# mmp/pbrt-v4

Hardware: AMD Instinct MI355X
Metric: Msamples/sec (whole node), 1920x1080 at fixed spp (higher is better)
Workload: dtype f32; 1 GPU; San Miguel 1080p 256spp (BASELINE.json configs[2]) on the sanmiguel-like stand-in at the SURVEY 8(d) spec: 10001008 unique triangles in 2000 meshes, 60 % of them in 200 object-instance definitions (two-level BVH), 10 % alpha-cut, 1k^2 image textures, diffuse / coated diffuse / dielectric / conductor, sun + 2k^2 image sky + 500 emitters, maxdepth 5, zsobol; step = 1 sample index x 1920x1080; spp=321, samples_per_pass=64, partition=single GPU

## Files before the change

### pbrt-v4_amd/csrc/hip/wf_backend.hip

```cpp
#include <hip/hip_runtime.h>
#include <array>

#include <climits>
#include <cstdarg>
#include <cstdio>
#include <cstring>
#include <algorithm>
#include <atomic>
#include <map>
#include <string>
#include <thread>
#include <type_traits>
#include <utility>
#include <vector>

#pragma clang attribute push(__attribute__((uninitialized)), apply_to = variable(is_local))
#include "../common/wf_kernels.h"
#include "../common/wf_kat.h"
#pragma clang attribute pop
#include "wf_traverse.h"

using namespace wf;

static thread_local char g_err[512] = "";
// ... 20 lines not shown
using ClosestWalkFn = void (*)(const SceneView, WorkState, FastBVH, int, SpillArea, int *, int, const int *);
using ShadowWalkFn = void (*)(const SceneView, WorkState, FastBVH, SpillArea, int *, int, const int *);
using TrTraceFn = void (*)(const SceneView, WorkState, FastBVH, int, SpillArea);
using TraceClosestFn = void (*)(const SceneView, FastBVH, int, const float *, wf_hit_record *, SpillArea);
using TraceAnyFn = void (*)(const SceneView, FastBVH, int, const float *, int32_t *, SpillArea);
struct WalkKernels {
    ClosestWalkFn closest = nullptr;
    ShadowWalkFn shadow = nullptr;
    ClosestWalkFn closestGen = nullptr;
    ShadowWalkFn shadowGen = nullptr;
    int grid = 1024, gridShadow = 1024, gridGen = 1024, gridShadowGen = 1024;
    TrTraceFn trTrace = nullptr;
    TraceClosestFn traceClosest = nullptr;
    TraceAnyFn traceAny = nullptr;
};

struct wf_ctx {
    int device = 0;
    hipStream_t stream = nullptr;
    std::vector<void *> allocs;
    SceneView svHost{};
    const SceneView *svDev = nullptr;
    WorkState ws{};
    int maxQueueSize = 0;
    int *stackSpill = nullptr;
    int spillRows = 0;
    int *dbgWords = nullptr;
    SpillArea spillArea() const { return SpillArea{stackSpill, spillRows, dbgWords}; }
    FastBVH fast{};
    bool fastOk = false;
    hipStream_t stream2 = nullptr;
    hipEvent_t evFork = nullptr, evJoin = nullptr;
    bool retracePending = false, deferJoin = false;
    int trWavefront = -1;
    bool cursorDirty[2] = {false, false};
    bool mediumLean = false;
    bool portalLights = false;
    bool leanShade = false;
    bool leanType[WF_MAT_NTYPES] = {};
    bool rareLights = false;
    int genMode = 0;
    bool deferGeneral = false;
    int genTri = 0;
    int nestedAnimated = 0;
    bool animFast = false;
    WalkKernels walk;
    int cursorChunk = 2;
    int cursorChunkShadow = 2;
    int32_t *probeCursor = nullptr;
    bool matPresent[WF_MAT_NTYPES] = {};
    int W = 0, H = 0;
    int maxDepth = 5;
    float sceneBounds[6] = {};
    bool sceneLoaded = false, queuesAllocated = false;
    int profile = 0;
    struct Ev { std::string name; hipEvent_t a, b; };
    std::vector<Ev> events;
    std::vector<hipEvent_t> eventPool;
    int passY0 = INT_MIN;
    int passStep = 1, passSamples = 1;
    bool pixelMajor = true;
    bool countTraversal = false;
    bool traceLaunch = false;
};

template <typename T>
static int devAlloc(wf_ctx *c, T **p, size_t n) {
    void *d = nullptr;
    size_t bytes = std::max<size_t>(n, 1) * sizeof(T);
    HIPCHK(hipMalloc(&d, bytes));
    HIPCHK(hipMemsetAsync(d, 0, bytes, c->stream));
    c->allocs.push_back(d);
    *p = (T *)d;
    return 0;
}
template <typename T>
static int devUpload(wf_ctx *c, const T **p, const T *src, size_t n) {
    T *d = nullptr;
    if (int e = devAlloc(c, &d, n)) return e;
    if (n && src) HIPCHK(hipMemcpyAsync(d, src, n * sizeof(T), hipMemcpyHostToDevice, c->stream));
    *p = d;
    return 0;
}

template <typename T>
static int devUpload(wf_ctx *c, wf::GPtr<const T> *p, const T *src, size_t n) {
    const T *d = nullptr;
    if (int e = devUpload(c, &d, src, n)) return e;
    *p = d;
    return 0;
}

template <bool VIA_SELF>
__device__ inline const SceneView &SvOf(const SceneView &a) { return VIA_SELF ? *a.self : a; }
__global__ void __launch_bounds__(BLOCK) k_reset(WorkState ws, unsigned mask, int statSlot, int statCounter) {
    if (threadIdx.x == 0 && blockIdx.x == 0) {
        if (statSlot >= 0) ws.stats[statSlot] += (unsigned long long)ws.counters[(statCounter) * CNT_STRIDE];
// ... 1082 lines not shown
}

struct Prof {
    wf_ctx *c;
    hipEvent_t a = nullptr, b = nullptr;
    const char *name;
    bool on;
    hipStream_t s;
    Prof(wf_ctx *c, const char *name, hipStream_t onStream = nullptr) : c(c), name(name), s(onStream ? onStream : c->stream) {
        if (c->traceLaunch) { fprintf(stderr, "[wf] launch %s\n", name); fflush(stderr); }
        on = c->profile == 1 || (c->profile == 2 && (strncmp(name, "Intersect", 9) == 0 || strcmp(name, "Route hits") == 0 || strstr(name, "Material") != nullptr ||
                                                      strncmp(name, "Sample medium", 13) == 0));
        if (!on) return;
        auto get = [&]() {
            hipEvent_t e;
            if (!c->eventPool.empty()) { e = c->eventPool.back(); c->eventPool.pop_back(); }
            else (void)hipEventCreate(&e);
            return e;
        };
        a = get(); b = get();
        (void)hipEventRecord(a, s);
    }
    ~Prof() {
        if (c->traceLaunch) {
            hipError_t e = hipStreamSynchronize(s);
            if (e != hipSuccess) { fprintf(stderr, "[wf] %s: %s\n", name, hipGetErrorString(e)); fflush(stderr); }
        }
        if (!on) return;
        (void)hipEventRecord(b, s);
        c->events.push_back({name, a, b});
    }
};

#define LAUNCH(name, kernel, grid, ...)                                                    \
    do {                                                                                   \
        Prof prof_(ctx, name);                                                             \
        hipLaunchKernelGGL(kernel, dim3(grid), dim3(BLOCK), 0, ctx->stream, __VA_ARGS__);  \
    } while (0)

#define LAUNCHT(name, kernel, grid, ...)                                                   \
    do {                                                                                   \
        Prof prof_(ctx, name);                                                             \
        hipLaunchKernelGGL(kernel, dim3(grid), dim3(TBLOCK), 0, ctx->stream, __VA_ARGS__); \
    } while (0)

static int statDepth(int depth) { return depth < 63 ? depth : 63; }

__global__ void k_pack_grid_corners(const float *v, int nx, int ny, int nz, float *out) {
    const size_t cells = (size_t)(nx + 1) * (ny + 1) * (nz + 1);
    for (size_t c = (size_t)blockIdx.x * blockDim.x + threadIdx.x; c < cells; c += (size_t)gridDim.x * blockDim.x) {
        const int cx = (int)(c % (size_t)(nx + 1)), cy = (int)((c / (size_t)(nx + 1)) % (size_t)(ny + 1)), cz = (int)(c / ((size_t)(nx + 1) * (ny + 1)));
        const int ix = cx - 1, iy = cy - 1, iz = cz - 1;
        float *o = out + 8 * wf::GridCornerIndex(nx, ny, cx, cy, cz);
        o[0] = wf::GridLookupI(v, nx, ny, nz, ix, iy, iz);         o[1] = wf::GridLookupI(v, nx, ny, nz, ix + 1, iy, iz);
        o[2] = wf::GridLookupI(v, nx, ny, nz, ix, iy + 1, iz);     o[3] = wf::GridLookupI(v, nx, ny, nz, ix + 1, iy + 1, iz);
        o[4] = wf::GridLookupI(v, nx, ny, nz, ix, iy, iz + 1);     o[5] = wf::GridLookupI(v, nx, ny, nz, ix + 1, iy, iz + 1);
        o[6] = wf::GridLookupI(v, nx, ny, nz, ix, iy + 1, iz + 1); o[7] = wf::GridLookupI(v, nx, ny, nz, ix + 1, iy + 1, iz + 1);
    }
}
static void useDevice(const wf_ctx *ctx) { (void)hipSetDevice(ctx->device); }
static int checkReady(wf_ctx *ctx) {
    if (!ctx) return fail(-1, "null context");
    if (!ctx->sceneLoaded) return fail(-1, "no scene uploaded");
    if (!ctx->queuesAllocated) return fail(-1, "queues not allocated (wf_queues_alloc)");
    useDevice(ctx);
    return 0;
}

struct FastDepths { int top = 0, def = 0, maxLeafInstances = 0; };
struct TopPrim {
    float b[6];
    int kind;
    int idx;
};
struct TopTreeBuilder {
    std::vector<TopPrim> &P;
    std::vector<wf_bvh_node> &out;
// ... 762 lines not shown
            const float(*mi)[4] = in.render_from_instance.mInv;
            double oI[3], dI[3];
            for (int a = 0; a < 3; ++a) {
                oI[a] = (double)mi[a][0] * o[0] + (double)mi[a][1] * o[1] + (double)mi[a][2] * o[2] + (double)mi[a][3];
                dI[a] = (double)mi[a][0] * dir[0] + (double)mi[a][1] * dir[1] + (double)mi[a][2] * dir[2];
            }
            const wf_instance_def &def = d->instance_defs[in.def];
            for (int k = def.first_prim; k < def.first_prim + def.n_prims; ++k)
                if (d->bvh_prims[k] < d->n_triangles) check(d->bvh_prims[k], ii, oI, dI);
        }
    }
    out[7] = cw.entries;
    out[3] = cw.nodesVisited;
    return 0;
}

constexpr int SCRATCH_PRIME_WORDS = 896;
__global__ void k_scratch_prime(int *out, int n) {
    volatile int buf[SCRATCH_PRIME_WORDS];
    for (int i = 0; i < n; ++i) buf[(i * 131) % SCRATCH_PRIME_WORDS] = i;
    out[threadIdx.x] = buf[(n * 7) % SCRATCH_PRIME_WORDS];
}
int wf_ctx_create(int device, wf_ctx **out) {
    if (!out) return fail(-1, "null out");
    int ndev = 0;
    HIPCHK(hipGetDeviceCount(&ndev));
    if (ndev <= 0) return fail(-1, "no HIP device visible: libwfhip has no CPU fallback");
    if (device < 0 || device >= ndev) return fail(-1, "device %d out of range (0..%d)", device, ndev - 1);
    HIPCHK(hipSetDevice(device));
    wf_ctx *c = new wf_ctx();
    c->device = device;
    HIPCHK(hipStreamCreateWithFlags(&c->stream, hipStreamNonBlocking));
    HIPCHK(hipStreamCreateWithFlags(&c->stream2, hipStreamNonBlocking));
    HIPCHK(hipEventCreateWithFlags(&c->evFork, hipEventDisableTiming));
    HIPCHK(hipEventCreateWithFlags(&c->evJoin, hipEventDisableTiming));
    c->traceLaunch = getenv("WF_TRACE_LAUNCH") != nullptr;
    if (const char *e = getenv("WF_SCRATCH_PRIME"); !e || atoi(e) != 0) {
        int *tmp = nullptr;
        HIPCHK(hipMalloc(&tmp, 64 * sizeof(int)));
        hipLaunchKernelGGL(k_scratch_prime, dim3(1), dim3(64), 0, c->stream, tmp, 8);
        hipLaunchKernelGGL(k_scratch_prime, dim3(1), dim3(64), 0, c->stream2, tmp, 8);
        HIPCHK(hipStreamSynchronize(c->stream));
        HIPCHK(hipStreamSynchronize(c->stream2));
        HIPCHK(hipFree(tmp));
    }
    *out = c;
    return 0;
}

int wf_ctx_destroy(wf_ctx *ctx) {
    if (!ctx) return 0;
    (void)hipSetDevice(ctx->device);
    (void)hipStreamSynchronize(ctx->stream);
    for (void *p : ctx->allocs) (void)hipFree(p);
    for (auto &e : ctx->events) { (void)hipEventDestroy(e.a); (void)hipEventDestroy(e.b); }
    for (auto e : ctx->eventPool) (void)hipEventDestroy(e);
    (void)hipStreamDestroy(ctx->stream);
    if (ctx->stream2) (void)hipStreamDestroy(ctx->stream2);
    if (ctx->evFork) (void)hipEventDestroy(ctx->evFork);
    if (ctx->evJoin) (void)hipEventDestroy(ctx->evJoin);
    delete ctx;
    return 0;
}

int wf_sync(wf_ctx *ctx) {
    if (!ctx) return fail(-1, "null context");
    useDevice(ctx);
    HIPCHK(hipStreamSynchronize(ctx->stream));
    HIPCHK(hipGetLastError());
    if (ctx->dbgWords) {
        int overflow = 0;
        HIPCHK(hipMemcpy(&overflow, ctx->dbgWords + 1, sizeof(int), hipMemcpyDeviceToHost));
        if (overflow) return fail(-1, "traversal stack overflow: a walk needed more than %d + %d node-stack entries (results are incomplete)", TSTACK, ctx->spillRows);
        int unresolved = 0;
        HIPCHK(hipMemcpy(&unresolved, ctx->dbgWords + 6, sizeof(int), hipMemcpyDeviceToHost));
        if (unresolved & 1) return fail(-1, "a near-tie re-walk found no hit where the production walk had one (results are incomplete)");
        if (unresolved & 2) return fail(-1, "a near-tie queue entry failed its validation (ray index, bound or launch tag): results are incomplete");
        int fatal = 0;
        HIPCHK(hipMemcpy(&fatal, ctx->dbgWords + 7, sizeof(int), hipMemcpyDeviceToHost));
        if (fatal) return fail(-1, "%s", FatalMessage(fatal));
        if (getenv("WF_DEBUG_DRAIN")) {
            int h[8];
            HIPCHK(hipMemcpy(h, ctx->dbgWords, sizeof(h), hipMemcpyDeviceToHost));
            fprintf(stderr, "[drain] spilled %d, re-walks %d, pushes %d, repeated re-walks %d, unresolved %d\n", h[0], h[2], h[4], h[5], h[6]);
#if WF_WALK_STATS
            unsigned long long c[16];
            HIPCHK(hipMemcpy(c, ctx->dbgWords + 8, sizeof(c), hipMemcpyDeviceToHost));
            const char *ph[4] = {"interior", "leaf", "transition", "refill"};
            for (int k = 0; k < 2; ++k)
                for (int q = 0; q < 4; ++q)
                    fprintf(stderr, "[walk stats] %s %-26s wave iterations %llu, lanes %llu (%.1f per iteration)\n", k ? "any-hit" : "closest", ph[q], c[k * 8 + 2 * q], c[k * 8 + 2 * q + 1],
// ... 275 lines not shown
                    st.pop_back();
                    best = std::max(best, dep);
                    if (d->bvh_nodes[i].nprims == 0) { st.push_back({i + 1, dep + 1}); st.push_back({d->bvh_nodes[i].offset, dep + 1}); }
                }
                return best;
            };
            int depthTop = d->n_bvh_nodes > 0 ? treeDepth(0) : 0, depthDef = 0;
            for (int k = 0; k < d->n_instance_defs; ++k) depthDef = std::max(depthDef, treeDepth(d->instance_defs[k].bvh_root));
            const int needRef = depthTop + (ctx->nestedAnimated > 0 ? 2 : 1) * depthDef + 4;
            const int needFast = 3 * fdep.top + fdep.maxLeafInstances + 3 * fdep.def + 6;
            const int rows = std::max(std::max(needRef - std::min(STACK_LDS, TSTACK), needFast - TSTACK), STACK_MAX - std::min(STACK_LDS, TSTACK));
            if (rows > 2048) return fail(-1, "BVH too deep for the traversal stacks (depth %d + %d)", depthTop, depthDef);
            if ((e = devAlloc(ctx, &ctx->stackSpill, (size_t)rows * MAX_GRID * BLOCK))) return e;
            ctx->spillRows = rows;
            if ((e = devAlloc(ctx, &ctx->dbgWords, (size_t)8 + 32))) return e;
            HIPCHK(hipMemset(ctx->dbgWords, 0, (8 + 32) * sizeof(int)));
        }
        if (ctx->fastOk) {
            if ((e = devUpload(ctx, &ctx->fast.nodes, qn.data(), qn.size()))) return e;
            if ((e = devUpload(ctx, &ctx->fast.tris, lt.data(), lt.size()))) return e;
            if ((e = devUpload(ctx, &ctx->fast.defs, fdefs.data(), fdefs.size()))) return e;
            if ((e = devUpload(ctx, &ctx->fast.subs, fsubs.data(), fsubs.size()))) return e;
            const bool big = qn.size() * sizeof(QNode) + lt.size() * sizeof(LeafTri) > ((size_t)256 << 20);
            ctx->cursorChunk = big ? 3 : 2;
            ctx->cursorChunkShadow = big ? 1 : 2;
            ctx->fast.instances = ctx->svHost.instances;
            HIPCHK(hipStreamSynchronize(ctx->stream));
        }
        if (getenv("WF_NO_FAST")) ctx->fastOk = false;
        ctx->animFast = d->n_animated > 0 && ctx->fastOk && ctx->genMode <= 1 && ctx->svHost.nInstances > 0 && !(getenv("WF_ANIM_FAST") && atoi(getenv("WF_ANIM_FAST")) == 0);
        if (d->n_animated > 0 && !ctx->animFast) ctx->fastOk = false;
        if ((e = PickWalkKernels(ctx))) return e;
        if ((e = devAlloc(ctx, &ctx->probeCursor, (size_t)1))) return e;
    }
    if ((e = devAlloc(ctx, &ctx->ws.film, (size_t)ctx->W * ctx->H * 4))) return e;
    ctx->ws.filmSpectral = nullptr;
    ctx->ws.filmGBuffer = nullptr;
    if (d->film.type == WF_FILM_GBUFFER && (e = devAlloc(ctx, &ctx->ws.filmGBuffer, (size_t)ctx->W * ctx->H))) return e;
    if (d->film.type == WF_FILM_SPECTRAL) {
        if (d->film.n_buckets < 1 || d->film.n_buckets > 4096 || !(d->film.lambda_max > d->film.lambda_min)) return fail(-1, "spectral film: bad bucket count / wavelength range");
        if ((e = devAlloc(ctx, &ctx->ws.filmSpectral, (size_t)ctx->W * ctx->H * 2 * d->film.n_buckets))) return e;
    }
    if ((e = devAlloc(ctx, &ctx->ws.stats, (size_t)(129 + 16)))) return e;
    if ((e = devAlloc(ctx, &ctx->ws.trav, (size_t)8))) return e;
    if ((e = devAlloc(ctx, &ctx->ws.counters, (size_t)CNT_COUNT * CNT_STRIDE))) return e;
    {
        SceneView *dev = nullptr;
        if ((e = devAlloc(ctx, &dev, (size_t)1))) return e;
        ctx->svHost.self = dev;
        ctx->svHost.fatal = ctx->dbgWords ? ctx->dbgWords + 7 : nullptr;
        HIPCHK(hipMemcpyAsync(dev, &ctx->svHost, sizeof(SceneView), hipMemcpyHostToDevice, ctx->stream));
        ctx->svDev = dev;
    }
    ctx->fast.sv = ctx->svDev;
    HIPCHK(hipStreamSynchronize(ctx->stream));
    ctx->sceneLoaded = true;
    return 0;
}

int wf_ctx_query(wf_ctx *ctx, const char *key, int64_t *value) {
    if (!ctx || !key || !value) return fail(-1, "wf_ctx_query: null argument");
    if (!ctx->sceneLoaded) return fail(-1, "no scene uploaded");
    const std::string k = key;
    if (k == "fast_ok") *value = ctx->fastOk;
    else if (k == "gen_mode") *value = ctx->genMode;
    else if (k == "gen_tri") *value = ctx->genTri;
    else if (k == "defer_general") *value = ctx->deferGeneral;
    else if (k == "anim_fast") *value = ctx->animFast;
    else if (k == "lean_shade") *value = ctx->leanShade;
    else if (k == "rare_lights") *value = ctx->rareLights;
    else if (k == "medium_lean") *value = ctx->mediumLean;
    else if (k.rfind("lean_type_", 0) == 0 && atoi(key + 10) >= 0 && atoi(key + 10) < WF_MAT_NTYPES) *value = ctx->leanType[atoi(key + 10)];
    else if (k == "instances") *value = ctx->svHost.nInstances;
    else if (k == "nested_animated") *value = ctx->nestedAnimated;
    else return fail(-1, "wf_ctx_query: unknown key '%s'", key);
    return 0;
}

int wf_aggregate_bounds(wf_ctx *ctx, float out_bounds[6]) {
    if (!ctx || !ctx->sceneLoaded) return fail(-1, "no scene uploaded");
    useDevice(ctx);
    for (int i = 0; i < 6; ++i) out_bounds[i] = ctx->sceneBounds[i];
    return 0;
}

static int allocRayQueue(wf_ctx *c, RayQueueV *q, size_t n) {
    int e;
    if ((e = devAlloc(c, &q->o, n)) || (e = devAlloc(c, &q->d, n)) || (e = devAlloc(c, &q->beta, n)) || (e = devAlloc(c, &q->r_u, n)) ||
        (e = devAlloc(c, &q->r_l, n)) || (e = devAlloc(c, &q->ctx0, n)) || (e = devAlloc(c, &q->ctx1, n)) || (e = devAlloc(c, &q->ctx2, n)) ||
        (e = devAlloc(c, &q->meta, n)))
        return e;
    return 0;
}

int wf_queues_alloc(wf_ctx *ctx, int pixels_per_pass, int samples_per_pass) {
    if (!ctx || !ctx->sceneLoaded) return fail(-1, "no scene uploaded");
    useDevice(ctx);
    if (ctx->queuesAllocated) return fail(-1, "queues already allocated");
    if (pixels_per_pass <= 0 || samples_per_pass <= 0) return fail(-1, "pixels_per_pass and samples_per_pass must be positive");
    if ((long long)pixels_per_pass * samples_per_pass > (1ll << 30)) return fail(-1, "queue capacity %lld too large", (long long)pixels_per_pass * samples_per_pass);
    if (pixels_per_pass % ctx->W != 0) return fail(-1, "pixels_per_pass must be a whole number of scanlines (width %d)", ctx->W);
    HIPCHK(hipSetDevice(ctx->device));
    const int max_queue_size = pixels_per_pass * samples_per_pass;
    const size_t n = (size_t)max_queue_size;
    WorkState &ws = ctx->ws;
    ws.maxQueueSize = max_queue_size;
    ws.pixelsPerPass = pixels_per_pass;
    ws.samplesPerPass = samples_per_pass;
    if (ws.stripCount < 1) { ws.stripRank = 0; ws.stripCount = 1; ws.stripHeight = 1; ws.localRows = ctx->H; }
    ctx->passSamples = 1;
    if (const char *e = getenv("WF_PIXEL_MAJOR")) ctx->pixelMajor = atoi(e) != 0;
    ctx->ws.slotStride = ctx->pixelMajor ? 1 : 0;
    ctx->passStep = 1;
    int e;
    if ((e = devAlloc(ctx, &ws.filterWeight, n)) || (e = devAlloc(ctx, &ws.pPixel, n)) || (e = devAlloc(ctx, &ws.lambda, n)) ||
        (e = devAlloc(ctx, &ws.lambdaPdf, n)) || (e = devAlloc(ctx, &ws.L, n)) || (e = devAlloc(ctx, &ws.cameraRayWeight, n)) ||
        (e = devAlloc(ctx, &ws.samples0, n)) || (e = devAlloc(ctx, &ws.samples1, n)))
        return e;
    if (ctx->svHost.film.type == WF_FILM_GBUFFER &&
        ((e = devAlloc(ctx, &ws.vsP, n)) || (e = devAlloc(ctx, &ws.vsN, n)) || (e = devAlloc(ctx, &ws.vsNs, n)) || (e = devAlloc(ctx, &ws.vsDpdx, n)) ||
         (e = devAlloc(ctx, &ws.vsDpdy, n)) || (e = devAlloc(ctx, &ws.vsAlbedo, n))))
        return e;
    ws.sampleTops = nullptr;
    if (ctx->svHost.sampler.type == WF_SAMPLER_ZSOBOL && 2 * ctx->svHost.sampler.nBase4Digits <= 32 && !getenv("WF_NO_SAMPLE_TOPS") &&
        !ctx->svHost.haveSubsurface)
        if ((e = devAlloc(ctx, &ws.sampleTops, (size_t)5 * pixels_per_pass))) return e;
    if ((e = allocRayQueue(ctx, &ws.rq[0], n)) || (e = allocRayQueue(ctx, &ws.rq[1], n))) return e;
    if (ctx->svHost.haveMedia) {
        if (getenv("WF_TR_WAVEFRONT")) ctx->trWavefront = atoi(getenv("WF_TR_WAVEFRONT"));
        if ((e = devAlloc(ctx, &ws.trO, n)) || (e = devAlloc(ctx, &ws.trD, n)) || (e = devAlloc(ctx, &ws.trT, n)) || (e = devAlloc(ctx, &ws.trRu, n)) ||
            (e = devAlloc(ctx, &ws.trRl, n)) || (e = devAlloc(ctx, &ws.trRng, n)) || (e = devAlloc(ctx, &ws.trQ[0], n)) || (e = devAlloc(ctx, &ws.trQ[1], n)))
            return e;
        if ((e = devAlloc(ctx, &ws.hitT, n)) || (e = devAlloc(ctx, &ws.mediumSampleQ, n)) || (e = devAlloc(ctx, &ws.mediumScatterQ, n)) || (e = devAlloc(ctx, &ws.mediumRouteQ, n)) ||
            (e = devAlloc(ctx, &ws.scatterP, n)) || (e = devAlloc(ctx, &ws.sq.medium, n)))
            return e;
    }
    if (ctx->svHost.haveMix && ((e = devAlloc(ctx, &ws.mixMat, n)) || (e = devAlloc(ctx, &ws.mixQ, n)))) return e;
    if (ctx->svHost.haveSubsurface && ((e = devAlloc(ctx, &ws.samples2, n)) || (e = devAlloc(ctx, &ws.bssrdfQ, n)) || (e = devAlloc(ctx, &ws.sssQ, n)))) return e;
    if ((e = devAlloc(ctx, &ws.hit, n)) || (e = devAlloc(ctx, &ws.escapedQ, n)) || (e = devAlloc(ctx, &ws.hitLightQ, n)) || (e = devAlloc(ctx, &ws.retraceQ, n)) || (e = devAlloc(ctx, &ws.retraceQ64, n))) return e;
    if ((e = devAlloc(ctx, &ws.deferQ, n))) return e;
    HIPCHK(hipMemset(ws.retraceQ64, 0xff, (size_t)n * sizeof(unsigned long long)));
    if (ctx->svHost.nInstances > 0 && (e = devAlloc(ctx, &ws.hitInst, n))) return e;
    for (int m = 0; m < WF_MAT_NTYPES; ++m)
        if ((e = devAlloc(ctx, &ws.matQ[m], ctx->matPresent[m] ? n : (size_t)1))) return e;
    if ((e = devAlloc(ctx, &ws.sq.o, n)) || (e = devAlloc(ctx, &ws.sq.d, n)) || (e = devAlloc(ctx, &ws.sq.Ld, n)) ||
        (e = devAlloc(ctx, &ws.sq.r_u, n)) || (e = devAlloc(ctx, &ws.sq.r_l, n)))
        return e;
    if (ctx->svHost.haveAnimated && (e = devAlloc(ctx, &ws.pathTime, n))) return e;
    {
        int planes = 0;
        for (int m = 1; m < WF_MAT_NTYPES; ++m) if (ctx->matPresent[m]) planes = std::max(planes, NeePlanes(m));
        if (planes > 0 && (e = devAlloc(ctx, &ws.neeRec, n * (size_t)planes))) return e;
    }
    if ((e = devAlloc(ctx, &ws.routeCode, n))) return e;
    ctx->maxQueueSize = max_queue_size;
    ctx->queuesAllocated = true;
    return 0;
}

int wf_set_pass_samples(wf_ctx *ctx, int sample_step, int n_samples) {
    if (int e = checkReady(ctx)) return e;
    if (n_samples < 1 || n_samples > ctx->ws.samplesPerPass) return fail(-1, "n_samples %d outside 1..%d", n_samples, ctx->ws.samplesPerPass);
    if (sample_step < 1) return fail(-1, "sample_step must be >= 1");
    ctx->passStep = sample_step;
    ctx->passSamples = n_samples;
    ctx->ws.slotStride = ctx->pixelMajor ? n_samples : 0;
    return 0;
}

int wf_set_strips(wf_ctx *ctx, int rank, int count, int height, int *local_rows) {
    if (!ctx || !ctx->sceneLoaded) return fail(-1, "no scene uploaded");
    useDevice(ctx);
    if (count < 1 || rank < 0 || rank >= count || height < 1) return fail(-1, "wf_set_strips: rank %d of %d, height %d", rank, count, height);
    int rows = 0;
    for (int y = 0; y < ctx->H; ++y) rows += (y / height) % count == rank;
    ctx->ws.stripRank = rank; ctx->ws.stripCount = count; ctx->ws.stripHeight = height; ctx->ws.localRows = count > 1 ? rows : ctx->H;
    if (local_rows) *local_rows = ctx->ws.localRows;
    return 0;
}

int wf_film_clear(wf_ctx *ctx) {
    if (!ctx || !ctx->sceneLoaded) return fail(-1, "no scene uploaded");
    useDevice(ctx);
    HIPCHK(hipMemsetAsync(ctx->ws.film, 0, (size_t)ctx->W * ctx->H * 4 * sizeof(double), ctx->stream));
    if (ctx->ws.filmGBuffer) HIPCHK(hipMemsetAsync(ctx->ws.filmGBuffer, 0, (size_t)ctx->W * ctx->H * sizeof(wf_gbuffer_pixel), ctx->stream));
    if (ctx->ws.filmSpectral) HIPCHK(hipMemsetAsync(ctx->ws.filmSpectral, 0, (size_t)ctx->W * ctx->H * 2 * ctx->svHost.film.n_buckets * sizeof(double), ctx->stream));
    HIPCHK(hipMemsetAsync(ctx->ws.stats, 0, (129 + 16) * sizeof(unsigned long long), ctx->stream));
    HIPCHK(hipMemsetAsync(ctx->ws.trav, 0, 8 * sizeof(unsigned long long), ctx->stream));
    return 0;
}

int wf_reset_ray_queue(wf_ctx *ctx, int which) {
    if (int e = checkReady(ctx)) return e;
    LAUNCH("Reset ray queue", k_reset, 1, ctx->ws, 1u << (CNT_RAY0 + (which & 1)), -1, 0);
    return 0;
}
int wf_reset_stage_queues(wf_ctx *ctx, int depth) {
    if (int e = checkReady(ctx)) return e;
    const int cur = depth & 1;
    unsigned mask = (1u << (CNT_RAY0 + (cur ^ 1))) | (1u << CNT_ESCAPED) | (1u << CNT_HITLIGHT);
    for (int m = 0; m < WF_MAT_NTYPES; ++m) mask |= 1u << (CNT_MAT0 + m);
    mask |= (1u << CNT_MEDIUM_SAMPLE) | (1u << CNT_MEDIUM_SCATTER) | (1u << CNT_MIX) | (1u << CNT_RETRACE) | (1u << CNT_BSSRDF) | (1u << CNT_SSS);
    mask |= (1u << CNT_RETRACE_HEAD) | (1u << CNT_WAVES_DONE) | (1u << CNT_CURSOR) | (1u << CNT_MEDIUM_ROUTE) | (1u << CNT_DEFER) | (1u << CNT_CURSOR_MEDIUM);
    LAUNCH("Reset queues before tracing rays", k_reset, 1, ctx->ws, mask, 1 + statDepth(depth), CNT_RAY0 + cur);
    ctx->cursorDirty[0] = false;
    return 0;
}
int wf_gen_camera_rays(wf_ctx *ctx, int y0, int sample_index) {
    if (int e = checkReady(ctx)) return e;
    ctx->passY0 = y0;
    if (ctx->ws.sampleTops) LAUNCH("Sampler index prefixes", k_sample_tops, gridFor(5 * ctx->ws.pixelsPerPass), ctx->svHost, ctx->ws, y0, 0);
    if (ctx->svHost.camera.type == WF_CAMERA_REALISTIC)
        LAUNCH("Reset ray queue", k_reset, 1, ctx->ws, 1u << CNT_RAY0, -1, 0);
    LAUNCH("Generate camera rays", (ctx->svHost.camera.anim.actually_animated ? k_gen_camera_rays<true> : k_gen_camera_rays<false>), gridFor(ctx->maxQueueSize), ctx->svHost, ctx->ws, y0, sample_index,
           ctx->passStep, ctx->passSamples);
    LAUNCH("Update camera ray stats", k_reset, 1, ctx->ws, 0u, 0, CNT_RAY0);
    return 0;
}
int wf_gen_ray_samples(wf_ctx *ctx, int depth, int sample_index) {
    if (int e = checkReady(ctx)) return e;
    const bool tops = ctx->ws.sampleTops != nullptr && ctx->passY0 != INT_MIN;
    if (tops) LAUNCH("Sampler index prefixes", k_sample_tops, gridFor(5 * ctx->ws.pixelsPerPass), ctx->svHost, ctx->ws, ctx->passY0, 6 + 7 * depth);
    LAUNCH("Generate ray samples - ZSobolSampler", k_gen_ray_samples, gridFor(ctx->maxQueueSize), ctx->svHost, ctx->ws, depth & 1, sample_index, ctx->passStep,
           tops ? depth : -1);
    return 0;
}
static int JoinRetrace(wf_ctx *ctx) {
    if (!ctx->retracePending) return 0;
    HIPCHK(hipStreamWaitEvent(ctx->stream, ctx->evJoin, 0));
    ctx->retracePending = false;
    return 0;
}
int wf_intersect_closest(wf_ctx *ctx, int depth) {
    if (int e = checkReady(ctx)) return e;
    const bool anim = ctx->svHost.haveAnimated;
    if (ctx->countTraversal)
// ... 86 lines not shown
                                               "DiffuseTransmissionMaterial + BxDF eval (Basic tex)", "CoatedDiffuseMaterial + BxDF eval (Basic tex)",
                                               "CoatedConductorMaterial + BxDF eval (Basic tex)", "SubsurfaceMaterial + BxDF eval (Basic tex)", "HairMaterial + BxDF eval (Basic tex)",
                                               "MeasuredMaterial + BxDF eval (Basic tex)"};
    if (material_type == WF_MAT_INTERFACE) return 0;
    if (material_type < 0 || material_type >= WF_MAT_NTYPES) return fail(-1, "material type %d has no HIP kernel", material_type);
    const bool tex = ctx->svHost.texNeedsFootprint != 0;
    const bool vs = ctx->svHost.film.type == WF_FILM_GBUFFER || ctx->svHost.camera.anim.actually_animated || ctx->svHost.haveAnimated ||
                    (ctx->svHost.haveCurves && ctx->svHost.haveQuadricAlpha);
    {
        Prof prof_(ctx, names[material_type]);
        const int v = vs ? 3 : (!ctx->leanType[material_type] ? 2 : (tex ? 1 : 0));
        kMatShade[material_type][v](ctx->stream, g, &ctx->svHost, &ctx->ws, cur);
    }
    {
        static const char *neeNames[WF_MAT_NTYPES] = {"", "DiffuseMaterial: next-event estimation", "ConductorMaterial: next-event estimation", "DielectricMaterial: next-event estimation",
                                                      "ThinDielectricMaterial: next-event estimation", "DiffuseTransmissionMaterial: next-event estimation",
                                                      "CoatedDiffuseMaterial: next-event estimation", "CoatedConductorMaterial: next-event estimation",
                                                      "SubsurfaceMaterial: next-event estimation", "HairMaterial: next-event estimation", "MeasuredMaterial: next-event estimation"};
        Prof prof_(ctx, neeNames[material_type]);
        kMatNee[material_type][ctx->rareLights ? 1 : 0](ctx->stream, g, &ctx->svHost, &ctx->ws);
    }
    return 0;
}
int wf_eval_material(wf_ctx *ctx, int material_type, int depth) {
    if (int e = checkReady(ctx)) return e;
    return EvalMaterial(ctx, material_type, depth);
}
static int EvalMaterials(wf_ctx *ctx, int depth) {
    for (int m = 1; m < WF_MAT_NTYPES; ++m)
        if (ctx->matPresent[m])
            if (int e = EvalMaterial(ctx, m, depth)) return e;
    return 0;
}
int wf_intersect_shadow(wf_ctx *ctx, int depth) {
    if (int e = checkReady(ctx)) return e;
    const bool anim = ctx->svHost.haveAnimated;
    if (ctx->countTraversal)
        LAUNCH("Intersect shadow", (anim ? k_intersect_shadow<true, true> : k_intersect_shadow<true, false>), gridFor(ctx->maxQueueSize), ctx->svHost, ctx->ws, ctx->stackSpill);
    else if (ctx->fastOk) {
        const WalkKernels &k = ctx->walk;
        int *cursor = ctx->ws.counters + CNT_CURSOR_SHADOW * CNT_STRIDE;
        if (ctx->cursorDirty[1]) HIPCHK(hipMemsetAsync(cursor, 0, sizeof(int), ctx->stream));
        ctx->cursorDirty[1] = true;
        LAUNCHT("Intersect shadow", k.shadow, k.gridShadow, ctx->svHost, ctx->ws, ctx->fast, ctx->spillArea(), cursor, ctx->cursorChunkShadow, (const int *)nullptr);
        if (k.shadowGen)
            LAUNCHT("Intersect shadow: rays that met a general primitive", k.shadowGen, k.gridShadowGen, ctx->svHost, ctx->ws, ctx->fast, ctx->spillArea(), (int *)nullptr, ctx->cursorChunkShadow, (const int *)ctx->ws.deferQ);
    } else
        LAUNCH("Intersect shadow", (anim ? k_intersect_shadow<false, true> : k_intersect_shadow<false, false>), gridFor(ctx->maxQueueSize), ctx->svHost, ctx->ws, ctx->stackSpill);
    LAUNCH("Reset shadowRayQueue", k_reset, 1, ctx->ws, (1u << CNT_SHADOW) | (1u << CNT_CURSOR_SHADOW) | (1u << CNT_DEFER_SHADOW), 65 + statDepth(depth), CNT_SHADOW);
    ctx->cursorDirty[1] = false;
    return 0;
}
int wf_subsurface_probe(wf_ctx *ctx, int depth) {
    if (int e = checkReady(ctx)) return e;
    if (!ctx->svHost.haveSubsurface) return 0;
    (void)depth;
    LAUNCH("Get BSSRDF and enqueue probe ray", k_subsurface_probe, gridFor(ctx->maxQueueSize), ctx->svHost, ctx->ws);
    return 0;
}
int wf_intersect_one_random(wf_ctx *ctx) {
    if (int e = checkReady(ctx)) return e;
    if (!ctx->svHost.haveSubsurface) return 0;
    LAUNCH("Intersect one random (subsurface probe)", (ctx->svHost.haveAnimated ? k_intersect_one_random<true> : k_intersect_one_random<false>), gridFor(ctx->maxQueueSize), ctx->svHost, ctx->ws, ctx->stackSpill);
    return 0;
}
int wf_subsurface_scatter(wf_ctx *ctx, int depth) {
    if (int e = checkReady(ctx)) return e;
    if (!ctx->svHost.haveSubsurface) return 0;
    LAUNCH("Handle out-scattering after SSS", k_subsurface_scatter, gridFor(ctx->maxQueueSize), ctx->svHost, ctx->ws, depth & 1);
    return 0;
}
int wf_update_film(wf_ctx *ctx) {
    if (int e = checkReady(ctx)) return e;
    if (ctx->ws.slotStride > 0 && ctx->ws.slotStride == ctx->passSamples && ctx->passSamples <= FILM_MAX_SLOTS && ctx->svHost.film.type == WF_FILM_RGB)
        LAUNCH("Update film", k_update_film_pm, std::min(4096, (ctx->ws.pixelsPerPass + FILM_PIX - 1) / FILM_PIX), ctx->svHost, ctx->ws, ctx->passSamples);
    else
        LAUNCH("Update film", k_update_film, gridFor(ctx->ws.pixelsPerPass), ctx->svHost, ctx->ws, ctx->passSamples);
    return 0;
}

int wf_render_pass(wf_ctx *ctx, int y0, int sample_index) {
    if (int e = checkReady(ctx)) return e;
    int e;
    if ((e = wf_reset_ray_queue(ctx, 0))) return e;
    if ((e = wf_gen_camera_rays(ctx, y0, sample_index))) return e;
    for (int depth = 0; true; ++depth) {
        if ((e = wf_reset_stage_queues(ctx, depth))) return e;
        ctx->deferJoin = ctx->fastOk && !ctx->countTraversal && !ctx->svHost.haveMix;
        if ((e = wf_intersect_closest(ctx, depth))) { ctx->deferJoin = false; return e; }
        ctx->deferJoin = false;
        if ((e = wf_gen_ray_samples(ctx, depth, sample_index))) return e;
        if ((e = JoinRetrace(ctx))) return e;
        if ((e = wf_medium_sample(ctx, depth))) return e;
        if ((e = wf_handle_escaped(ctx, depth))) return e;
        if ((e = wf_handle_emissive(ctx, depth))) return e;
        if (depth == ctx->maxDepth) break;
        if ((e = EvalMaterials(ctx, depth))) return e;
        if ((e = ctx->svHost.haveMedia ? wf_intersect_shadow_tr(ctx, depth) : wf_intersect_shadow(ctx, depth))) return e;
        if (ctx->svHost.haveSubsurface) {
            if ((e = wf_subsurface_probe(ctx, depth)) || (e = wf_intersect_one_random(ctx)) || (e = wf_subsurface_scatter(ctx, depth))) return e;
            if ((e = ctx->svHost.haveMedia ? wf_intersect_shadow_tr(ctx, depth) : wf_intersect_shadow(ctx, depth))) return e;
        }
    }
    return wf_update_film(ctx);
}

int wf_film_download(wf_ctx *ctx, double *dst) {
    if (!ctx || !ctx->sceneLoaded) return fail(-1, "no scene uploaded");
    useDevice(ctx);
    HIPCHK(hipMemcpyAsync(dst, ctx->ws.film, (size_t)ctx->W * ctx->H * 4 * sizeof(double), hipMemcpyDeviceToHost, ctx->stream));
    HIPCHK(hipStreamSynchronize(ctx->stream));
    return 0;
}
int wf_film_spectral_download(wf_ctx *ctx, double *dst) {
    if (!ctx || !ctx->sceneLoaded) return fail(-1, "no scene uploaded");
    useDevice(ctx);
    if (!ctx->ws.filmSpectral) return fail(-1, "wf_film_spectral_download: the scene's film is not a spectral film");
    HIPCHK(hipMemcpyAsync(dst, ctx->ws.filmSpectral, (size_t)ctx->W * ctx->H * 2 * ctx->svHost.film.n_buckets * sizeof(double), hipMemcpyDeviceToHost, ctx->stream));
    HIPCHK(hipStreamSynchronize(ctx->stream));
    return 0;
}
int wf_film_gbuffer_download(wf_ctx *ctx, wf_gbuffer_pixel *dst) {
    if (!ctx || !ctx->sceneLoaded) return fail(-1, "no scene uploaded");
    useDevice(ctx);
    if (!ctx->ws.filmGBuffer) return fail(-1, "wf_film_gbuffer_download: the scene's film is not a gbuffer film");
    HIPCHK(hipMemcpyAsync(dst, ctx->ws.filmGBuffer, (size_t)ctx->W * ctx->H * sizeof(wf_gbuffer_pixel), hipMemcpyDeviceToHost, ctx->stream));
    HIPCHK(hipStreamSynchronize(ctx->stream));
    return 0;
}
int wf_film_upload(wf_ctx *ctx, const double *src) {
    if (!ctx || !ctx->sceneLoaded) return fail(-1, "no scene uploaded");
    useDevice(ctx);
    HIPCHK(hipMemcpyAsync(ctx->ws.film, src, (size_t)ctx->W * ctx->H * 4 * sizeof(double), hipMemcpyHostToDevice, ctx->stream));
    HIPCHK(hipStreamSynchronize(ctx->stream));
    return 0;
}
int wf_film_device_ptr(wf_ctx *ctx, void **dptr, uint64_t *nbytes) {
// ... 490 lines not shown
```

Baseline: 439.0 Msamples/s.

## Overlap shadow-ray tracing with next-depth closest-hit on a third stream

Moves the shadow-ray intersection stage onto a separate stream with its own spill buffer and defer queue, so it runs alongside the next bounce's closest-hit traversal. The join is deferred until after ray-sample generation. Stage-queue resets are restricted so they never zero the shadow counters. Separately, ray-sample generation is skipped at the final depth when no media or subsurface need it. The overlap adds memory for a second spill area and depends on the shadow and closest-hit kernels not conflicting on shared state.

```diff
diff --git a/pbrt-v4_amd/csrc/hip/wf_backend.hip b/pbrt-v4_amd/csrc/hip/wf_backend.hip
--- a/pbrt-v4_amd/csrc/hip/wf_backend.hip
+++ b/pbrt-v4_amd/csrc/hip/wf_backend.hip
@@ -76,6 +76,13 @@
     hipStream_t stream2 = nullptr;
     hipEvent_t evFork = nullptr, evJoin = nullptr;
     bool retracePending = false, deferJoin = false;
+    hipStream_t stream3 = nullptr;
+    hipEvent_t evShadowFork = nullptr, evShadowJoin = nullptr;
+    int frameOverlap = 1;
+    bool shadowPending = false;
+    int *stackSpill2 = nullptr;
+    int32_t *deferQShadow = nullptr;
+    bool samplesShaded = true;
     int trWavefront = -1;
     bool cursorDirty[2] = {false, false};
     bool mediumLean = false;
@@ -107,6 +114,11 @@
     bool countTraversal = false;
     bool traceLaunch = false;
 };
+
+static bool FrameOverlapScene(const wf_ctx *ctx) {
+    return ctx->frameOverlap > 0 && ctx->fastOk && !ctx->svHost.haveMedia && !ctx->svHost.haveSubsurface && !ctx->svHost.haveAnimated;
+}
+constexpr int FRAME_OVERLAP_THIN_DEPTH = 2;
 
 template <typename T>
 static int devAlloc(wf_ctx *c, T **p, size_t n) {
@@ -1255,17 +1267,19 @@
     }
 };
 
-#define LAUNCH(name, kernel, grid, ...)                                                    \
+#define LAUNCH_ON(strm, name, kernel, grid, ...)                                           \
     do {                                                                                   \
-        Prof prof_(ctx, name);                                                             \
-        hipLaunchKernelGGL(kernel, dim3(grid), dim3(BLOCK), 0, ctx->stream, __VA_ARGS__);  \
+        Prof prof_(ctx, name, strm);                                                       \
+        hipLaunchKernelGGL(kernel, dim3(grid), dim3(BLOCK), 0, strm, __VA_ARGS__);         \
     } while (0)
-
-#define LAUNCHT(name, kernel, grid, ...)                                                   \
+#define LAUNCH(name, kernel, grid, ...) LAUNCH_ON(ctx->stream, name, kernel, grid, __VA_ARGS__)
+
+#define LAUNCHT_ON(strm, name, kernel, grid, ...)                                          \
     do {                                                                                   \
-        Prof prof_(ctx, name);                                                             \
-        hipLaunchKernelGGL(kernel, dim3(grid), dim3(TBLOCK), 0, ctx->stream, __VA_ARGS__); \
+        Prof prof_(ctx, name, strm);                                                       \
+        hipLaunchKernelGGL(kernel, dim3(grid), dim3(TBLOCK), 0, strm, __VA_ARGS__);        \
     } while (0)
+#define LAUNCHT(name, kernel, grid, ...) LAUNCHT_ON(ctx->stream, name, kernel, grid, __VA_ARGS__)
 
 static int statDepth(int depth) { return depth < 63 ? depth : 63; }
 
@@ -2094,16 +2108,23 @@
     c->device = device;
     HIPCHK(hipStreamCreateWithFlags(&c->stream, hipStreamNonBlocking));
     HIPCHK(hipStreamCreateWithFlags(&c->stream2, hipStreamNonBlocking));
+    HIPCHK(hipStreamCreateWithFlags(&c->stream3, hipStreamNonBlocking));
     HIPCHK(hipEventCreateWithFlags(&c->evFork, hipEventDisableTiming));
     HIPCHK(hipEventCreateWithFlags(&c->evJoin, hipEventDisableTiming));
+    HIPCHK(hipEventCreateWithFlags(&c->evShadowFork, hipEventDisableTiming));
+    HIPCHK(hipEventCreateWithFlags(&c->evShadowJoin, hipEventDisableTiming));
+    if (const char *e = getenv("WF_FRAME_OVERLAP")) c->frameOverlap = std::min(2, std::max(0, atoi(e)));
+    if (const char *e = getenv("WF_SAMPLES_SHADED")) c->samplesShaded = atoi(e) != 0;
     c->traceLaunch = getenv("WF_TRACE_LAUNCH") != nullptr;
     if (const char *e = getenv("WF_SCRATCH_PRIME"); !e || atoi(e) != 0) {
         int *tmp = nullptr;
         HIPCHK(hipMalloc(&tmp, 64 * sizeof(int)));
         hipLaunchKernelGGL(k_scratch_prime, dim3(1), dim3(64), 0, c->stream, tmp, 8);
         hipLaunchKernelGGL(k_scratch_prime, dim3(1), dim3(64), 0, c->stream2, tmp, 8);
+        hipLaunchKernelGGL(k_scratch_prime, dim3(1), dim3(64), 0, c->stream3, tmp, 8);
         HIPCHK(hipStreamSynchronize(c->stream));
         HIPCHK(hipStreamSynchronize(c->stream2));
+        HIPCHK(hipStreamSynchronize(c->stream3));
         HIPCHK(hipFree(tmp));
     }
     *out = c;
@@ -2114,11 +2135,15 @@
     if (!ctx) return 0;
     (void)hipSetDevice(ctx->device);
     (void)hipStreamSynchronize(ctx->stream);
+    if (ctx->stream3) (void)hipStreamSynchronize(ctx->stream3);
     for (void *p : ctx->allocs) (void)hipFree(p);
     for (auto &e : ctx->events) { (void)hipEventDestroy(e.a); (void)hipEventDestroy(e.b); }
     for (auto e : ctx->eventPool) (void)hipEventDestroy(e);
     (void)hipStreamDestroy(ctx->stream);
     if (ctx->stream2) (void)hipStreamDestroy(ctx->stream2);
+    if (ctx->stream3) (void)hipStreamDestroy(ctx->stream3);
+    if (ctx->evShadowFork) (void)hipEventDestroy(ctx->evShadowFork);
+    if (ctx->evShadowJoin) (void)hipEventDestroy(ctx->evShadowJoin);
     if (ctx->evFork) (void)hipEventDestroy(ctx->evFork);
     if (ctx->evJoin) (void)hipEventDestroy(ctx->evJoin);
     delete ctx;
@@ -2460,6 +2485,7 @@
         if (d->n_animated > 0 && !ctx->animFast) ctx->fastOk = false;
         if ((e = PickWalkKernels(ctx))) return e;
         if ((e = devAlloc(ctx, &ctx->probeCursor, (size_t)1))) return e;
+        if (FrameOverlapScene(ctx) && (e = devAlloc(ctx, &ctx->stackSpill2, (size_t)ctx->spillRows * MAX_GRID * BLOCK))) return e;
     }
     if ((e = devAlloc(ctx, &ctx->ws.film, (size_t)ctx->W * ctx->H * 4))) return e;
     ctx->ws.filmSpectral = nullptr;
@@ -2501,6 +2527,9 @@
     else if (k.rfind("lean_type_", 0) == 0 && atoi(key + 10) >= 0 && atoi(key + 10) < WF_MAT_NTYPES) *value = ctx->leanType[atoi(key + 10)];
     else if (k == "instances") *value = ctx->svHost.nInstances;
     else if (k == "nested_animated") *value = ctx->nestedAnimated;
+    else if (k == "frame_overlap_active") *value = FrameOverlapScene(ctx) && ctx->stackSpill2 != nullptr;
+    else if (k == "frame_overlap_mode") *value = ctx->frameOverlap;
+    else if (k == "skip_last_samples") *value = ctx->samplesShaded && !ctx->svHost.haveMedia && !ctx->svHost.haveSubsurface;
     else return fail(-1, "wf_ctx_query: unknown key '%s'", key);
     return 0;
 }
@@ -2567,6 +2596,7 @@
     if (ctx->svHost.haveSubsurface && ((e = devAlloc(ctx, &ws.samples2, n)) || (e = devAlloc(ctx, &ws.bssrdfQ, n)) || (e = devAlloc(ctx, &ws.sssQ, n)))) return e;
     if ((e = devAlloc(ctx, &ws.hit, n)) || (e = devAlloc(ctx, &ws.escapedQ, n)) || (e = devAlloc(ctx, &ws.hitLightQ, n)) || (e = devAlloc(ctx, &ws.retraceQ, n)) || (e = devAlloc(ctx, &ws.retraceQ64, n))) return e;
     if ((e = devAlloc(ctx, &ws.deferQ, n))) return e;
+    if (ctx->stackSpill2 && ctx->walk.shadowGen && (e = devAlloc(ctx, &ctx->deferQShadow, n))) return e;
     HIPCHK(hipMemset(ws.retraceQ64, 0xff, (size_t)n * sizeof(unsigned long long)));
     if (ctx->svHost.nInstances > 0 && (e = devAlloc(ctx, &ws.hitInst, n))) return e;
     for (int m = 0; m < WF_MAT_NTYPES; ++m)
@@ -2626,10 +2656,13 @@
 int wf_reset_stage_queues(wf_ctx *ctx, int depth) {
     if (int e = checkReady(ctx)) return e;
     const int cur = depth & 1;
-    unsigned mask = (1u << (CNT_RAY0 + (cur ^ 1))) | (1u << CNT_ESCAPED) | (1u << CNT_HITLIGHT);
-    for (int m = 0; m < WF_MAT_NTYPES; ++m) mask |= 1u << (CNT_MAT0 + m);
-    mask |= (1u << CNT_MEDIUM_SAMPLE) | (1u << CNT_MEDIUM_SCATTER) | (1u << CNT_MIX) | (1u << CNT_RETRACE) | (1u << CNT_BSSRDF) | (1u << CNT_SSS);
-    mask |= (1u << CNT_RETRACE_HEAD) | (1u << CNT_WAVES_DONE) | (1u << CNT_CURSOR) | (1u << CNT_MEDIUM_ROUTE) | (1u << CNT_DEFER) | (1u << CNT_CURSOR_MEDIUM);
+    constexpr unsigned matBits = ((1u << WF_MAT_NTYPES) - 1u) << CNT_MAT0;
+    constexpr unsigned stageMask = (1u << CNT_ESCAPED) | (1u << CNT_HITLIGHT) | matBits |
+        (1u << CNT_MEDIUM_SAMPLE) | (1u << CNT_MEDIUM_SCATTER) | (1u << CNT_MIX) | (1u << CNT_RETRACE) | (1u << CNT_BSSRDF) | (1u << CNT_SSS) |
+        (1u << CNT_RETRACE_HEAD) | (1u << CNT_WAVES_DONE) | (1u << CNT_CURSOR) | (1u << CNT_MEDIUM_ROUTE) | (1u << CNT_DEFER) | (1u << CNT_CURSOR_MEDIUM);
+    static_assert((stageMask & ((1u << CNT_SHADOW) | (1u << CNT_CURSOR_SHADOW) | (1u << CNT_DEFER_SHADOW))) == 0 && CNT_SHADOW != CNT_RAY0 && CNT_SHADOW != CNT_RAY1,
+                  "the stage reset must not zero a counter of the shadow stage, which may be running beside it");
+    const unsigned mask = stageMask | (1u << (CNT_RAY0 + (cur ^ 1)));
     LAUNCH("Reset queues before tracing rays", k_reset, 1, ctx->ws, mask, 1 + statDepth(depth), CNT_RAY0 + cur);
     ctx->cursorDirty[0] = false;
     return 0;
@@ -2782,23 +2815,43 @@
             if (int e = EvalMaterial(ctx, m, depth)) return e;
     return 0;
 }
+static int ShadowStage(wf_ctx *ctx, int depth, hipStream_t strm, int *spill) {
+    const bool anim = ctx->svHost.haveAnimated;
+    if (ctx->countTraversal)
+        LAUNCH_ON(strm, "Intersect shadow", (anim ? k_intersect_shadow<true, true> : k_intersect_shadow<true, false>), gridFor(ctx->maxQueueSize), ctx->svHost, ctx->ws, spill);
+    else if (ctx->fastOk) {
+        const WalkKernels &k = ctx->walk;
+        const SpillArea area{spill, ctx->spillRows, ctx->dbgWords};
+        int *cursor = ctx->ws.counters + CNT_CURSOR_SHADOW * CNT_STRIDE;
+        if (ctx->cursorDirty[1]) HIPCHK(hipMemsetAsync(cursor, 0, sizeof(int), strm));
+        ctx->cursorDirty[1] = true;
+        WorkState ws = ctx->ws;
+        if (strm != ctx->stream && ctx->deferQShadow) ws.deferQ = ctx->deferQShadow;
+        LAUNCHT_ON(strm, "Intersect shadow", k.shadow, k.gridShadow, ctx->svHost, ws, ctx->fast, area, cursor, ctx->cursorChunkShadow, (const int *)nullptr);
+        if (k.shadowGen)
+            LAUNCHT_ON(strm, "Intersect shadow: rays that met a general primitive", k.shadowGen, k.gridShadowGen, ctx->svHost, ws, ctx->fast, area, (int *)nullptr, ctx->cursorChunkShadow, (const int *)ws.deferQ);
+    } else
+        LAUNCH_ON(strm, "Intersect shadow", (anim ? k_intersect_shadow<false, true> : k_intersect_shadow<false, false>), gridFor(ctx->maxQueueSize), ctx->svHost, ctx->ws, spill);
+    LAUNCH_ON(strm, "Reset shadowRayQueue", k_reset, 1, ctx->ws, (1u << CNT_SHADOW) | (1u << CNT_CURSOR_SHADOW) | (1u << CNT_DEFER_SHADOW), 65 + statDepth(depth), CNT_SHADOW);
+    ctx->cursorDirty[1] = false;
+    return 0;
+}
 int wf_intersect_shadow(wf_ctx *ctx, int depth) {
     if (int e = checkReady(ctx)) return e;
-    const bool anim = ctx->svHost.haveAnimated;
-    if (ctx->countTraversal)
-        LAUNCH("Intersect shadow", (anim ? k_intersect_shadow<true, true> : k_intersect_shadow<true, false>), gridFor(ctx->maxQueueSize), ctx->svHost, ctx->ws, ctx->stackSpill);
-    else if (ctx->fastOk) {
-        const WalkKernels &k = ctx->walk;
-        int *cursor = ctx->ws.counters + CNT_CURSOR_SHADOW * CNT_STRIDE;
-        if (ctx->cursorDirty[1]) HIPCHK(hipMemsetAsync(cursor, 0, sizeof(int), ctx->stream));
-        ctx->cursorDirty[1] = true;
-        LAUNCHT("Intersect shadow", k.shadow, k.gridShadow, ctx->svHost, ctx->ws, ctx->fast, ctx->spillArea(), cursor, ctx->cursorChunkShadow, (const int *)nullptr);
-        if (k.shadowGen)
-            LAUNCHT("Intersect shadow: rays that met a general primitive", k.shadowGen, k.gridShadowGen, ctx->svHost, ctx->ws, ctx->fast, ctx->spillArea(), (int *)nullptr, ctx->cursorChunkShadow, (const int *)ctx->ws.deferQ);
-    } else
-        LAUNCH("Intersect shadow", (anim ? k_intersect_shadow<false, true> : k_intersect_shadow<false, false>), gridFor(ctx->maxQueueSize), ctx->svHost, ctx->ws, ctx->stackSpill);
-    LAUNCH("Reset shadowRayQueue", k_reset, 1, ctx->ws, (1u << CNT_SHADOW) | (1u << CNT_CURSOR_SHADOW) | (1u << CNT_DEFER_SHADOW), 65 + statDepth(depth), CNT_SHADOW);
-    ctx->cursorDirty[1] = false;
+    return ShadowStage(ctx, depth, ctx->stream, ctx->stackSpill);
+}
+static int IssueShadowAside(wf_ctx *ctx, int depth) {
+    HIPCHK(hipEventRecord(ctx->evShadowFork, ctx->stream));
+    HIPCHK(hipStreamWaitEvent(ctx->stream3, ctx->evShadowFork, 0));
+    if (int e = ShadowStage(ctx, depth, ctx->stream3, ctx->stackSpill2)) return e;
+    HIPCHK(hipEventRecord(ctx->evShadowJoin, ctx->stream3));
+    ctx->shadowPending = true;
+    return 0;
+}
+static int JoinShadow(wf_ctx *ctx) {
+    if (!ctx->shadowPending) return 0;
+    HIPCHK(hipStreamWaitEvent(ctx->stream, ctx->evShadowJoin, 0));
+    ctx->shadowPending = false;
     return 0;
 }
 int wf_subsurface_probe(wf_ctx *ctx, int depth) {
@@ -2829,9 +2882,10 @@
     return 0;
 }
 
-int wf_render_pass(wf_ctx *ctx, int y0, int sample_index) {
-    if (int e = checkReady(ctx)) return e;
+static int RenderPass(wf_ctx *ctx, int y0, int sample_index) {
     int e;
+    const bool aside = ctx->stackSpill2 != nullptr && FrameOverlapScene(ctx) && ctx->profile != 1 && !ctx->traceLaunch && !ctx->countTraversal;
+    const bool skipLastSamples = ctx->samplesShaded && !ctx->svHost.haveMedia && !ctx->svHost.haveSubsurface;
     if ((e = wf_reset_ray_queue(ctx, 0))) return e;
     if ((e = wf_gen_camera_rays(ctx, y0, sample_index))) return e;
     for (int depth = 0; true; ++depth) {
@@ -2839,20 +2893,35 @@
         ctx->deferJoin = ctx->fastOk && !ctx->countTraversal && !ctx->svHost.haveMix;
         if ((e = wf_intersect_closest(ctx, depth))) { ctx->deferJoin = false; return e; }
         ctx->deferJoin = false;
-        if ((e = wf_gen_ray_samples(ctx, depth, sample_index))) return e;
+        if (!(skipLastSamples && depth == ctx->maxDepth) && (e = wf_gen_ray_samples(ctx, depth, sample_index))) return e;
         if ((e = JoinRetrace(ctx))) return e;
+        if ((e = JoinShadow(ctx))) return e;
         if ((e = wf_medium_sample(ctx, depth))) return e;
         if ((e = wf_handle_escaped(ctx, depth))) return e;
         if ((e = wf_handle_emissive(ctx, depth))) return e;
         if (depth == ctx->maxDepth) break;
         if ((e = EvalMaterials(ctx, depth))) return e;
+        if (aside && (ctx->frameOverlap == 1 || depth >= FRAME_OVERLAP_THIN_DEPTH)) {
+            if ((e = IssueShadowAside(ctx, depth))) return e;
+            continue;
+        }
         if ((e = ctx->svHost.haveMedia ? wf_intersect_shadow_tr(ctx, depth) : wf_intersect_shadow(ctx, depth))) return e;
         if (ctx->svHost.haveSubsurface) {
             if ((e = wf_subsurface_probe(ctx, depth)) || (e = wf_intersect_one_random(ctx)) || (e = wf_subsurface_scatter(ctx, depth))) return e;
             if ((e = ctx->svHost.haveMedia ? wf_intersect_shadow_tr(ctx, depth) : wf_intersect_shadow(ctx, depth))) return e;
         }
     }
+    if ((e = JoinShadow(ctx))) return e;
     return wf_update_film(ctx);
+}
+int wf_render_pass(wf_ctx *ctx, int y0, int sample_index) {
+    if (int e = checkReady(ctx)) return e;
+    const int e = RenderPass(ctx, y0, sample_index);
+    if (e) {
+        (void)hipStreamSynchronize(ctx->stream3);
+        ctx->shadowPending = false;
+    }
+    return e;
 }
 
 int wf_film_download(wf_ctx *ctx, double *dst) {
```

After: 448.1 Msamples/s (median of 6 runs). 2.1% higher.
